# QEDProtocol/plonky2.5

Measured on AMD Instinct MI355X. Metric: recursive proofs/sec (fib-64 p3-in-p2 circuit), higher is better.
Workload: dtype u64 (Goldilocks, p = 2^64 - 2^32 + 1); 1 GPU; batch of 256 independent fib-64 plonky3-verifier proofs per GPU (n = 2^16 rows x 135 wires, LDE 2^19), 1 GPU(s), replicas + RCCL gather; all_statuses_ok=True, gathered_complete_and_ok=True, head=

## Files before the change

plonky2.5_amd/csrc/kernels.h:

```cpp
#pragma once
#include <hip/hip_runtime.h>
#include <stddef.h>
#include <stdint.h>
#include <stdexcept>
#include <string>
#include <vector>
#include <map>
#include <tuple>
#include "dev_res.h"
#include "gl.h"

#if defined(__HIP_DEVICE_COMPILE__)
#define P25_WAVE_PRIO(n) __builtin_amdgcn_s_setprio(n)
#else
#define P25_WAVE_PRIO(n) ((void)0)
#endif
#define P25_PRIO_BULK 2
#define P25_PRIO_CHAIN 3
namespace p25 {

void launch_poseidon_permute(u64* d_states, size_t n, hipStream_t st);
void launch_poseidon2_permute(u64* d_states, size_t n, hipStream_t st);
size_t merkle_tree_words(size_t n_leaves, unsigned cap_height);
size_t merkle_level_offset(size_t n_leaves, unsigned level);
u64* launch_merkle_tree(const u64* d_cols, size_t col_stride, int width, size_t n_leaves,
                        unsigned cap_height, u64* d_tree, hipStream_t st, hipEvent_t ev_begin = nullptr,
                        hipEvent_t ev_end = nullptr, bool single_proof = false);

struct NttPass {
  const u64* in;
  u64* out;
  size_t in_poly_stride, out_poly_stride;
  size_t coset_out_off[8];
  int log_r, log_nt, log_t;
  int in_kind, in_br_t, in_br_i;
  int out_kind, out_br_t, out_br_i;
  const u64* pow_table;
  int log_n_table;
  int use_twiddle;
  const u64* pre;
  const u64* pre_t;
  const u64* pre_i;
  const u64* post_t;
  const u64* post_i;
  int inverse;
  int lazy_out;
  uint32_t n_tiles, n_cosets, log_g, full_table;
};
void launch_ntt_pass(const NttPass& p, int n_polys, int n_cosets, hipStream_t st);
double measure_shader_clock_hz(hipStream_t st);

class NttTables {
 public:
  const u64* pow_table(int log_n, bool inverse);
  const u64* geom_table(u64 first, u64 ratio, size_t len);
  const u64* upload(const std::vector<u64>& host);
  typedef std::map<std::tuple<int, int, u64>, const u64*> CosetCache;
  CosetCache& coset_cache() { return coset_; }

 private:
  CosetCache coset_;
  std::map<std::pair<int, bool>, u64*> pow_;
  std::map<std::tuple<u64, u64, size_t>, u64*> geom_;
  std::vector<DevMem> owned_;
};

void ntt_inverse(NttTables& tb, const u64* d_in, size_t in_stride, bool in_bitrev, u64* d_tmp,
                 size_t tmp_stride, u64* d_out, size_t out_stride, int log_n, int n_polys,
                 u64 coset_shift, hipStream_t st);
void ntt_lde_bitrev(NttTables& tb, const u64* d_coeffs, size_t coeff_stride, u64* d_lde,
                    size_t lde_stride, int log_n, int rate_bits, int n_polys, u64 shift,
                    hipStream_t st);

void ntt_inverse_then_lde(NttTables& tb, const u64* d_vals, size_t val_stride, u64* d_tmp, size_t tmp_stride, u64* d_coeffs,
                          size_t coeff_stride, u64* d_lde, size_t lde_stride, int log_n, int rate_bits, int n_polys, u64 shift,
                          hipStream_t st);

}
```

plonky2.5_amd/csrc/kernels_fri.hip:

```cpp
#include "kernels.h"
#include "gl_lazy.h"
#include "coop.h"
#include "coop_lat.h"
#include "poseidon.h"
#include "prover_kernels.h"

namespace p25 {

constexpr uint32_t EXT_POW_MAX_JOBS = 5;
struct ExtPowJob {
  const u64* point;
  u64 scale;
  u64* out;
  uint32_t count, invert;
};
struct ExtPowJobs {
  ExtPowJob job[EXT_POW_MAX_JOBS];
};
__global__ void k_ext_pows(ExtPowJobs a) {
  P25_WAVE_PRIO(P25_PRIO_CHAIN);
  const ExtPowJob jb = a.job[blockIdx.y];
  uint32_t t = blockIdx.x * blockDim.x + threadIdx.x;
  if (t > jb.count) return;
  gl::E2 z = gl::mul(gl::E2{jb.point[0], jb.point[1]}, jb.scale);
// ... 138 lines not shown
  gl::E2 s0 = gl::e2(0);
  uint32_t j = 0;
  for (int o = 0; o < 4; o++)
    for (uint32_t p = 0; p < a.n_polys[o]; p++, j++) {
      u64 c = a.coeffs[o][(size_t)p * n + k];
      s0.a = gl::mad_nc(ap[2 * j], c, s0.a);
      s0.b = gl::mad_nc(ap[2 * j + 1], c, s0.b);
    }
  gl::E2 s1 = gl::e2(0);
  for (uint32_t c = 0; c < a.num_challenges; c++) {
    u64 v = a.coeffs[2][(size_t)c * n + k];
    s1.a = gl::mad_nc(ap[2 * c], v, s1.a);
    s1.b = gl::mad_nc(ap[2 * c + 1], v, s1.b);
  }
  gl::E2 d0 = gl::e2_canon(gl::e2_mul_nc(s0, gl::E2{a.zpow[0][2 * k], a.zpow[0][2 * k + 1]}));
  gl::E2 d1 = gl::e2_canon(gl::e2_mul_nc(s1, gl::E2{a.zpow[1][2 * k], a.zpow[1][2 * k + 1]}));
  a.comp[0 * (size_t)n + k] = d0.a;
  a.comp[1 * (size_t)n + k] = d0.b;
  a.comp[2 * (size_t)n + k] = d1.a;
  a.comp[3 * (size_t)n + k] = d1.b;
}

__global__ __launch_bounds__(256) void k_sfx_block(u64* data, uint32_t n, u64* block_tot) {
  P25_WAVE_PRIO(P25_PRIO_CHAIN);
  __shared__ u64 sh[256];
  u64* d = data + (size_t)blockIdx.y * n;
  uint32_t i = blockIdx.x * 256 + threadIdx.x;
  u64 v = i < n ? d[n - 1 - i] : 0;
  sh[threadIdx.x] = v;
  __syncthreads();
  for (int off = 1; off < 256; off <<= 1) {
    u64 t = threadIdx.x >= (unsigned)off ? sh[threadIdx.x - off] : 0;
    __syncthreads();
    v = gl::add(v, t);
    sh[threadIdx.x] = v;
    __syncthreads();
  }
  u64 ex = threadIdx.x == 0 ? 0 : sh[threadIdx.x - 1];
  if (i < n) d[n - 1 - i] = ex;
  if (threadIdx.x == 255) block_tot[(size_t)blockIdx.y * gridDim.x + blockIdx.x] = v;
}
__global__ __launch_bounds__(256) void k_sfx_totals(u64* block_tot, uint32_t n_blocks) {
  P25_WAVE_PRIO(P25_PRIO_CHAIN);
  __shared__ u64 sh[256];
  __shared__ u64 carry_s;
  u64* bt = block_tot + (size_t)blockIdx.x * n_blocks;
  if (threadIdx.x == 0) carry_s = 0;
  __syncthreads();
  for (uint32_t base = 0; base < n_blocks; base += 256) {
    uint32_t i = base + threadIdx.x;
    u64 v = i < n_blocks ? bt[i] : 0;
    sh[threadIdx.x] = v;
    __syncthreads();
    for (int off = 1; off < 256; off <<= 1) {
      u64 t = threadIdx.x >= (unsigned)off ? sh[threadIdx.x - off] : 0;
      __syncthreads();
      v = gl::add(v, t);
      sh[threadIdx.x] = v;
      __syncthreads();
    }
    u64 carry = carry_s;
    u64 excl = threadIdx.x == 0 ? carry : gl::add(carry, sh[threadIdx.x - 1]);
    __syncthreads();
    if (i < n_blocks) bt[i] = excl;
    if (threadIdx.x == 255) carry_s = gl::add(carry, v);
    __syncthreads();
  }
}
__global__ __launch_bounds__(256) void k_sfx_apply(u64* data, uint32_t n, const u64* block_tot) {
  P25_WAVE_PRIO(P25_PRIO_CHAIN);
  u64* d = data + (size_t)blockIdx.y * n;
  uint32_t i = blockIdx.x * 256 + threadIdx.x;
  if (i >= n) return;
  d[n - 1 - i] = gl::add(d[n - 1 - i], block_tot[(size_t)blockIdx.y * gridDim.x + blockIdx.x]);
}

__global__ __launch_bounds__(256) void k_fri_final(const u64* __restrict__ S, uint32_t n,
                                                   const u64* __restrict__ zinv0, const u64* __restrict__ zinv1,
                                                   const u64* __restrict__ alpha_pows, uint32_t nc,
                                                   u64* __restrict__ fa, u64* __restrict__ fb) {
  P25_WAVE_PRIO(P25_PRIO_CHAIN);
  uint32_t k = blockIdx.x * blockDim.x + threadIdx.x;
  if (k >= n) return;
  if (k == n - 1) {
    fa[0] = 0;
    fb[0] = 0;
    return;
  }
  gl::E2 q0 = gl::mul(gl::E2{S[k], S[(size_t)n + k]}, gl::E2{zinv0[2 * (k + 1)], zinv0[2 * (k + 1) + 1]});
  gl::E2 q1 = gl::mul(gl::E2{S[2 * (size_t)n + k], S[3 * (size_t)n + k]}, gl::E2{zinv1[2 * (k + 1)], zinv1[2 * (k + 1) + 1]});
  gl::E2 f = gl::add(gl::mul(q0, gl::E2{alpha_pows[2 * nc], alpha_pows[2 * nc + 1]}), q1);
  fa[k + 1] = f.a;
  fb[k + 1] = f.b;
}

void launch_fri_combine(const FriCombineArgs& a, hipStream_t st) {
  const uint32_t n = 1u << a.log_n;
  uint32_t total = a.n_polys[0] + a.n_polys[1] + a.n_polys[2] + a.n_polys[3];
  u64* alpha_pows = a.scan_tmp;
  u64* zpow0 = alpha_pows + 2 * (size_t)(total + 1);
  u64* zpow1 = zpow0 + 2 * (size_t)(n + 1);
  u64* zinv0 = zpow1 + 2 * (size_t)(n + 1);
  u64* zinv1 = zinv0 + 2 * (size_t)(n + 1);
  u64* block_tot = zinv1 + 2 * (size_t)(n + 1);
  const unsigned nb = (n + 255) / 256;
  ExtPowJobs pj{};
  pj.job[0] = ExtPowJob{a.chal + CH_FRI_ALPHA, (u64)1, alpha_pows, total, 0};
  pj.job[1] = ExtPowJob{a.chal + CH_ZETA, (u64)1, zpow0, n, 0};
  pj.job[2] = ExtPowJob{a.chal + CH_ZETA, a.g, zpow1, n, 0};
  pj.job[3] = ExtPowJob{a.chal + CH_ZETA, (u64)1, zinv0, n, 1};
  pj.job[4] = ExtPowJob{a.chal + CH_ZETA, a.g, zinv1, n, 1};
  launch_ext_pows(pj, 5, st);
  CombineK ck;
  for (int o = 0; o < 4; o++) {
    ck.coeffs[o] = a.coeffs[o];
    ck.n_polys[o] = a.n_polys[o];
  }
  ck.log_n = a.log_n;
  ck.num_challenges = a.num_challenges;
  ck.alpha_pows = alpha_pows;
  ck.zpow[0] = zpow0;
  ck.zpow[1] = zpow1;
  ck.comp = a.comp;
  hipLaunchKernelGGL(k_fri_comp, dim3(nb), dim3(256), 2 * total * sizeof(u64), st, ck);
  hipLaunchKernelGGL(k_sfx_block, dim3(nb, 4), dim3(256), 0, st, a.comp, n, block_tot);
  hipLaunchKernelGGL(k_sfx_totals, dim3(4), dim3(256), 0, st, block_tot, nb);
  hipLaunchKernelGGL(k_sfx_apply, dim3(nb, 4), dim3(256), 0, st, a.comp, n, block_tot);
  hipLaunchKernelGGL(k_fri_final, dim3(nb), dim3(256), 0, st, a.comp, n, zinv0, zinv1, alpha_pows, a.num_challenges, a.final_a, a.final_b);
}

__global__ __launch_bounds__(256) void k_fri_fold(const u64* __restrict__ ca, const u64* __restrict__ cb,
                                                  uint32_t len_out, uint32_t arity_bits,
                                                  const u64* __restrict__ beta, u64* __restrict__ oa,
                                                  u64* __restrict__ ob) {
  P25_WAVE_PRIO(P25_PRIO_BULK);
  uint32_t i = blockIdx.x * blockDim.x + threadIdx.x;
  if (i >= len_out) return;
  const uint32_t arity = 1u << arity_bits;
  gl::E2 b{beta[0], beta[1]};
  gl::E2 s = gl::e2(0);
  for (int k = (int)arity - 1; k >= 0; k--) {
    s = gl::mul(s, b);
    s = gl::add(s, gl::E2{ca[(size_t)i * arity + k], cb[(size_t)i * arity + k]});
  }
  oa[i] = s.a;
  ob[i] = s.b;
}
void launch_fri_fold(const u64* ca, const u64* cb, uint32_t len_out, uint32_t arity_bits, const u64* d_beta,
                     u64* oa, u64* ob, hipStream_t st) {
  hipLaunchKernelGGL(k_fri_fold, dim3((len_out + 255) / 256), dim3(256), 0, st, ca, cb, len_out, arity_bits, d_beta, oa, ob);
}

template <int PRIO>
__global__ __launch_bounds__(256) void k_fri_leaf_hash(const u64* __restrict__ va, const u64* __restrict__ vb,
                                                       uint32_t n_leaves, uint32_t arity_bits,
                                                       u64* __restrict__ digests) {
  if constexpr (PRIO != 0) P25_WAVE_PRIO(PRIO);
  uint32_t l = blockIdx.x * blockDim.x + threadIdx.x;
  if (l >= n_leaves) return;
  const uint32_t arity = 1u << arity_bits, words = 2 * arity;
  u64 s[12];
#pragma unroll
  for (int i = 0; i < 12; i++) s[i] = 0;
  u64 out[4];
  if (words <= 4) {
    for (uint32_t i = 0; i < 4; i++) out[i] = i < words ? ((i & 1) ? vb : va)[(size_t)l * arity + (i >> 1)] : 0;
  } else {
    for (uint32_t off = 0; off < words; off += 8) {
      uint32_t m = words - off < 8 ? words - off : 8;
      for (uint32_t i = 0; i < m; i++) {
        uint32_t wd = off + i;
        s[i] = ((wd & 1) ? vb : va)[(size_t)l * arity + (wd >> 1)];
      }
      poseidon::permute(s);
    }
    for (int i = 0; i < 4; i++) out[i] = s[i];
  }
  for (int i = 0; i < 4; i++) digests[4 * (size_t)l + i] = out[i];
}
__global__ __launch_bounds__(256) void k_fri_leaf_hash_coop(const u64* __restrict__ va, const u64* __restrict__ vb,
                                                            uint32_t n_leaves, uint32_t arity_bits,
                                                            u64* __restrict__ digests) {
  P25_WAVE_PRIO(P25_PRIO_CHAIN);
  __shared__ u64 rc_lds[360];
  coop::stage_poseidon_rc(rc_lds);
  size_t g = ((size_t)blockIdx.x * blockDim.x + threadIdx.x) / coop::GROUP;
  const int rr = threadIdx.x & (coop::GROUP - 1);
  const bool valid = g < n_leaves;
  if (!valid) g = n_leaves - 1;
  const uint32_t arity = 1u << arity_bits, words = 2 * arity;
  u64 s = 0;
  for (uint32_t off = 0; off < words; off += 8) {
    const uint32_t m = words - off < 8 ? words - off : 8;
    const uint32_t wd = off + (uint32_t)rr;
    if ((uint32_t)rr < m) s = ((wd & 1) ? vb : va)[g * arity + (wd >> 1)];
    s = coop::poseidon_permute_lat(s, threadIdx.x & 63, rc_lds);
  }
  if (valid && rr < 4) digests[4 * g + rr] = s;
}
constexpr uint32_t COOP_FRI_LEAVES_BATCH = 2048;
constexpr int FRI_LEAF_PRIO_BATCH = 1;
void launch_fri_leaf_hash(const u64* va, const u64* vb, uint32_t n_leaves, uint32_t arity_bits, u64* d_digests,
                          hipStream_t st, bool single_proof) {
  const bool noop = (2u << arity_bits) <= 4;
  if (single_proof ? noop : (noop || n_leaves > COOP_FRI_LEAVES_BATCH)) {
    if (single_proof)
      hipLaunchKernelGGL(k_fri_leaf_hash<0>, dim3((n_leaves + 255) / 256), dim3(256), 0, st, va, vb, n_leaves, arity_bits,
                         d_digests);
    else
      hipLaunchKernelGGL(k_fri_leaf_hash<FRI_LEAF_PRIO_BATCH>, dim3((n_leaves + 63) / 64), dim3(64), 0, st, va, vb, n_leaves,
                         arity_bits, d_digests);
    return;
  }
  const size_t th = (size_t)n_leaves * coop::GROUP;
  hipLaunchKernelGGL(k_fri_leaf_hash_coop, dim3((unsigned)((th + 255) / 256)), dim3(256), 0, st, va, vb, n_leaves,
                     arity_bits, d_digests);
}

__device__ __forceinline__ size_t level_off(size_t n_leaves, uint32_t k) { return 8 * n_leaves - ((8 * n_leaves) >> k); }

__global__ __launch_bounds__(256) void k_queries(QueryArgs a) {
  P25_WAVE_PRIO(P25_PRIO_CHAIN);
  const uint32_t q = blockIdx.x, t = threadIdx.x, nt = blockDim.x;
  const size_t big = (size_t)1 << a.lde_bits;
  size_t x = (size_t)(a.chal[CH_QUERIES + q] & (big - 1));
  u64* out = a.proof + a.query_offset + (size_t)q * a.query_stride;
  const uint32_t path_len = a.lde_bits - a.cap_height;
  for (uint32_t o = 0; o < a.n_oracles; o++) {
    for (uint32_t c = t; c < a.oracle_width[o]; c += nt) out[c] = a.oracle_lde[o][(size_t)c * big + x];
    out += a.oracle_width[o];
    for (uint32_t e = t; e < 4 * path_len; e += nt) {
      uint32_t k = e >> 2;
      out[e] = a.oracle_tree[o][level_off(big, k) + 4 * ((x >> k) ^ 1) + (e & 3)];
    }
    out += 4 * path_len;
  }
  uint32_t bits = a.lde_bits;
  for (uint32_t l = 0; l < a.n_layers; l++) {
    const uint32_t ab = a.arity_bits[l], arity = 1u << ab;
    bits -= ab;
    const size_t n_leaves = (size_t)1 << bits;
    const size_t ci = x >> ab;
    for (uint32_t e = t; e < 2 * arity; e += nt) out[e] = ((e & 1) ? a.layer_vb[l] : a.layer_va[l])[ci * arity + (e >> 1)];
    out += 2 * arity;
    const uint32_t pl = bits - a.cap_height;
    for (uint32_t e = t; e < 4 * pl; e += nt) {
      uint32_t k = e >> 2;
      out[e] = a.layer_tree[l][level_off(n_leaves, k) + 4 * ((ci >> k) ^ 1) + (e & 3)];
    }
    out += 4 * pl;
    x = ci;
  }
}
void launch_queries(const QueryArgs& a, hipStream_t st) {
  hipLaunchKernelGGL(k_queries, dim3(a.num_queries), dim3(256), 0, st, a);
}

}
```

plonky2.5_amd/csrc/kernels_quotient.hip:

```cpp
#include <stdexcept>
#include <stdlib.h>
#include "builder.h"
#include "kernels.h"
#include "gl_lazy.h"
#include "poseidon.h"
#include "poseidon2.h"
#include "coop.h"
#include "prover_kernels.h"

namespace p25 {

namespace {

struct AlphaLimbs {
  u32 l[8];
};
constexpr int MAX_TERMS_PER_FOLD = 512;

struct LaneCols {
  const u64* base;
  u32 boff;
  size_t big;
  typedef unsigned int u32x2 __attribute__((ext_vector_type(2)));
  __device__ __forceinline__ u64 col(size_t c) const {
// ... 371 lines not shown
  for (int copy = 0; copy < RA_COPIES; copy++) {
    const int base = (2 + RA_VEC) * copy;
    u64 bits[RA_BITS];
    for (int i = 0; i < RA_BITS; i++) {
      bits[i] = cx.w(RA_ROUTED + RA_BITS * copy + i);
      cx.at(nc++, gl::mul_nc(bits[i], gl::sub(bits[i], 1)));
    }
    u64 idx = 0;
    for (int i = RA_BITS - 1; i >= 0; i--) idx = gl::add(gl::add(idx, idx), bits[i]);
    cx.at(nc++, gl::sub(idx, cx.w(base)));
    u64 items[RA_VEC];
    for (int i = 0; i < RA_VEC; i++) items[i] = cx.w(base + 2 + i);
    int len = RA_VEC;
    for (int bi = 0; bi < RA_BITS; bi++) {
      len >>= 1;
      for (int i = 0; i < len; i++)
        items[i] = gl::add(items[2 * i], gl::mul(bits[bi], gl::sub(items[2 * i + 1], items[2 * i])));
    }
    cx.at(nc++, gl::sub(items[0], cx.w(base + 1)));
  }
  cx.at(nc++, gl::sub(k0, cx.w((2 + RA_VEC) * RA_COPIES)));
  cx.at(nc++, gl::sub(k1, cx.w((2 + RA_VEC) * RA_COPIES + 1)));
}
template <bool EXT>
__device__ void gate_reducing(Ctx& cx) {
  constexpr int NCO = EXT ? REDX_COEFFS : RED_COEFFS, CW = EXT ? 2 : 1, START_ACCS = 6 + NCO * CW;
  const gl::E2 alpha{cx.w(2), cx.w(3)};
  gl::E2 acc{cx.w(4), cx.w(5)};
  auto acc_wire = [](int i) { return i == NCO - 1 ? 0 : START_ACCS + 2 * i; };
  u64 na = cx.w(acc_wire(0)), nb = cx.w(acc_wire(0) + 1), nc0 = cx.w(6), nc1 = EXT ? cx.w(7) : 0;
  for (int i = 0; i < NCO; i++) {
    const gl::E2 nxt{na, nb};
    const u64 c0 = nc0, c1 = nc1;
    if (i + 1 < NCO) {
      na = cx.w(acc_wire(i + 1));
      nb = cx.w(acc_wire(i + 1) + 1);
      nc0 = cx.w(6 + CW * (i + 1));
      if (EXT) nc1 = cx.w(6 + CW * (i + 1) + 1);
    }
    gl::E2 t = gl::mul(acc, alpha);
    t.a = gl::add(t.a, c0);
    if (EXT) t.b = gl::add(t.b, c1);
    cx.at(2 * i, gl::sub(t.a, nxt.a));
    cx.at(2 * i + 1, gl::sub(t.b, nxt.b));
    acc = nxt;
  }
}
__device__ void gate_poseidon_mds(Ctx& cx) {
  for (int d = 0; d < 2; d++) {
    u64 in[12];
#pragma unroll
    for (int i = 0; i < 12; i++) in[i] = cx.w(2 * i + d);
    u64 nxt = cx.w(24 + d);
#pragma unroll
    for (int r = 0; r < 12; r++) {
      const u64 o = nxt;
      if (r + 1 < 12) nxt = cx.w(24 + 2 * (r + 1) + d);
      SmallLin acc;
#pragma unroll
      for (int i = 0; i < 12; i++) acc.add(in[(i + r) % 12], (u32)poseidon::MDS_CIRC[i] + (i == 0 && r == 0 ? (u32)poseidon::MDS_DIAG0 : 0u));
      cx.at(2 * r + d, gl::sub(o, gl::canon(acc.value())));
    }
  }
}
__device__ void gate_coset_interp(Ctx& cx) {
  const u64 shift = cx.w(0);
  const gl::E2 point{cx.w(CI_W_POINT), cx.w(CI_W_POINT + 1)}, x{cx.w(CI_W_SHIFTED), cx.w(CI_W_SHIFTED + 1)};
  int nc = 0;
  cx.at(nc++, gl::sub(point.a, gl::mul(x.a, shift)));
  cx.at(nc++, gl::sub(point.b, gl::mul(x.b, shift)));
  const u64 g = gl::root_of_unity(4), inv16 = gl::inv(16);
  gl::E2 eval{0, 0}, prod{1, 0};
  u64 xi = 1;
  for (int c = 0; c <= CI_INTER; c++) {
    if (c > 0) {
      const gl::E2 ie{cx.w(CI_W_INTER + 2 * (c - 1)), cx.w(CI_W_INTER + 2 * (c - 1) + 1)};
      const gl::E2 ip{cx.w(CI_W_INTER + 2 * (CI_INTER + c - 1)), cx.w(CI_W_INTER + 2 * (CI_INTER + c - 1) + 1)};
      cx.at(nc++, gl::sub(ie.a, eval.a));
      cx.at(nc++, gl::sub(ie.b, eval.b));
      cx.at(nc++, gl::sub(ip.a, prod.a));
      cx.at(nc++, gl::sub(ip.b, prod.b));
      eval = ie;
      prod = ip;
    }
    const int end = c == 0 ? CI_DEGREE : (1 + (CI_DEGREE - 1) * (c + 1) < CI_POINTS ? 1 + (CI_DEGREE - 1) * (c + 1) : CI_POINTS);
    for (int i = c == 0 ? 0 : 1 + (CI_DEGREE - 1) * c; i < end; i++) {
      const gl::E2 v = gl::mul(gl::E2{cx.w(1 + 2 * i), cx.w(2 + 2 * i)}, gl::mul(xi, inv16));
      const gl::E2 term{gl::sub(x.a, xi), x.b};
      eval = gl::add(gl::mul(eval, term), gl::mul(v, prod));
      prod = gl::mul(prod, term);
      xi = gl::mul(xi, g);
    }
  }
  cx.at(nc++, gl::sub(cx.w(CI_W_VALUE), eval.a));
  cx.at(nc++, gl::sub(cx.w(CI_W_VALUE + 1), eval.b));
}
__device__ void gate_poseidon(Ctx& cx) {
  int nc = 0;
  u64 swap = cx.w(24);
  cx.at(nc++, gl::mul_nc(swap, gl::sub(swap, 1)));
  u64 st[12];
#pragma unroll
  for (int i = 0; i < 4; i++) {
    u64 lhs = cx.w(i), rhs = cx.w(i + 4), delta = cx.w(25 + i);
    cx.at(nc++, gl::sub(gl::mul(swap, gl::sub(rhs, lhs)), delta));
    st[i] = gl::add(lhs, delta);
    st[i + 4] = gl::sub(rhs, delta);
  }
#pragma unroll
  for (int i = 8; i < 12; i++) st[i] = cx.w(i);
  int tr = 29;
  u64 nsb = cx.w(tr);
  constexpr int TR_END = 29 + 12 * (2 * poseidon::HALF_FULL - 1) + poseidon::N_PARTIAL;
  for (int r = 0; r < poseidon::N_ROUNDS; r++) {
#pragma unroll
    for (int i = 0; i < 12; i++) st[i] = poseidon::add_rc(st[i], poseidon::RC[12 * r + i]);
    if (r < poseidon::HALF_FULL || r >= poseidon::HALF_FULL + poseidon::N_PARTIAL) {
      if (r != 0) {
#pragma unroll
        for (int i = 0; i < 12; i++) {
          const u64 sb = nsb;
          tr++;
          if (tr < TR_END) nsb = cx.w(tr);
          cx.at(nc++, gl::sub(gl::canon(st[i]), sb));
          st[i] = sb;
        }
      }
#pragma unroll
      for (int i = 0; i < 12; i++) st[i] = poseidon::sbox(st[i]);
    } else {
      const u64 sb = nsb;
      tr++;
      if (tr < TR_END) nsb = cx.w(tr);
      cx.at(nc++, gl::sub(gl::canon(st[0]), sb));
      st[0] = poseidon::sbox(sb);
    }
    poseidon::mds(st);
  }
#pragma unroll
  for (int i = 0; i < 12; i++) cx.at(nc++, gl::sub(gl::canon(st[i]), cx.w(12 + i)));
}

}

__global__ void k_alpha_pows(const u64* __restrict__ chal, u64* __restrict__ out) {
  P25_WAVE_PRIO(P25_PRIO_CHAIN);
  int c = blockIdx.x, j = threadIdx.x;
  if (j < ALPHA_POWS) out[c * ALPHA_POWS + j] = gl::pow(chal[CH_ALPHAS + c], (u64)j);
}
void launch_alpha_pows(const u64* d_chal, u64* d_alpha_pows, hipStream_t st) {
  hipLaunchKernelGGL(k_alpha_pows, dim3(2), dim3(ALPHA_POWS), 0, st, d_chal, d_alpha_pows);
}

constexpr int Q_WAVES = 4;
constexpr int QREC_WAVES = 3;
constexpr int Q_PF = 1;
template <bool REC>
__device__ __forceinline__ void quotient_body(const QuotientArgs& a) {
  __shared__ u64 ap[2 * ALPHA_POWS];
  __shared__ AlphaLimbs apl[ALPHA_POWS];
  for (int i = threadIdx.x; i < 2 * ALPHA_POWS; i += blockDim.x) {
    const u64 v = a.alpha_pows[i];
    ap[i] = v;
    const int ch = i / ALPHA_POWS, j = i - ch * ALPHA_POWS;
    apl[j].l[4 * ch] = (u32)v & 0x3FFFFFu;
    apl[j].l[4 * ch + 1] = (u32)(v >> 22) & 0x3FFFFFu;
    apl[j].l[4 * ch + 2] = (u32)(v >> 44);
    apl[j].l[4 * ch + 3] = 0;
  }
  __shared__ u64 kb[2 * MAX_ROUTED];
  for (int i = threadIdx.x; i < 2 * (int)a.num_routed; i += blockDim.x) {
    const int c = i / (int)a.num_routed, j = i - c * (int)a.num_routed;
    kb[i] = gl::mul(a.k_is[j], a.chal[CH_BETAS + c]);
  }
  __syncthreads();
  const uint32_t lde_bits = a.degree_bits + a.rate_bits;
  const size_t big = (size_t)1 << lde_bits;
  const size_t p = (size_t)blockIdx.x * blockDim.x + threadIdx.x;
  if (p >= big) return;
  const uint32_t i_nat = gl::bitrev((u32)p, lde_bits);
  const u64 x = gl::mul(gl::GENERATOR, a.pow_big[i_nat]);
  const uint32_t rate_mask = (1u << a.rate_bits) - 1;
  const u64 zhx = a.zh[i_nat & rate_mask], zhi = a.zh_inv[i_nat & rate_mask];
  const uint32_t i_next = (i_nat + (1u << a.rate_bits)) & (uint32_t)(big - 1);
  const size_t p_next = gl::bitrev(i_next, lde_bits);

  const int NC = 2, NP = (int)a.num_partial_products, RW = (int)a.num_routed;
  const int nch = NP + 1, per = (int)a.quotient_degree_factor;
  const u32 boff = (u32)p * 8u;
  const LaneCols csc{a.cs_lde, boff, big}, wrc{a.wires_lde, boff, big}, zsc{a.zs_lde, boff, big};
  const int n_consts = (int)a.num_selectors;

  u64 res[2] = {0, 0};
  {
    u64 l0 = gl::mul_nc(zhx, a.l0_inv[p]);
    for (int c = 0; c < NC; c++) {
      u64 t = gl::mul_nc(l0, gl::sub_c(zsc.col(c), 1));
      res[0] = gl::mad_nc(t, ap[c], res[0]);
      res[1] = gl::mad_nc(t, ap[ALPHA_POWS + c], res[1]);
    }
  }
  auto gate_filter = [&](uint32_t gi) {
    const GateEntry ge = a.gates[gi];
    const u64 s = csc.col(ge.selector_index);
    u64 filter = 1;
    for (uint32_t k = ge.group_start; k < ge.group_end; k++)
      if (k != gi) filter = gl::mul_nc(filter, gl::sub_c((u64)k, s));
    if (a.num_selectors > 1) filter = gl::mul_nc(filter, gl::sub_c(0xFFFFFFFFull, s));
    return filter;
  };
  const bool fast = per == 8 && RW == 80 && NP == 9 && a.num_wires >= 80;
  uint32_t merged_mask = 0;
  u64 mg0 = 0, mg1 = 0;
  const u64 beta0 = a.chal[CH_BETAS], beta1 = a.chal[CH_BETAS + 1];
  const u64 gamma0 = a.chal[CH_GAMMAS], gamma1 = a.chal[CH_GAMMAS + 1];
  if (fast) {
    for (uint32_t gi = 0; gi < a.n_gates; gi++) {
      const uint32_t kind = a.gates[gi].kind;
      if (kind == G_CONSTANT || kind == G_PUBLIC_INPUT || kind == G_BASE_SUM || kind == G_ARITHMETIC || kind == G_MUL_EXT) {
        if ((merged_mask >> kind) & 1u) { merged_mask = 0xFFFFFFFFu; break; }
        merged_mask |= 1u << kind;
      }
    }
  }
  if (fast && merged_mask != 0xFFFFFFFFu) {
    const bool h_const = (merged_mask >> G_CONSTANT) & 1u, h_pi = (merged_mask >> G_PUBLIC_INPUT) & 1u,
               h_bsum = (merged_mask >> G_BASE_SUM) & 1u, h_arith = (merged_mask >> G_ARITHMETIC) & 1u,
               h_mext = (merged_mask >> G_MUL_EXT) & 1u;
    u64 f_const = 0, f_pi = 0, f_bsum = 0, f_arith = 0, f_mext = 0;
    for (uint32_t gi = 0; gi < a.n_gates; gi++) {
      const uint32_t kind = a.gates[gi].kind;
      if (kind == G_CONSTANT) f_const = gate_filter(gi);
      else if (kind == G_PUBLIC_INPUT) f_pi = gate_filter(gi);
      else if (kind == G_BASE_SUM) f_bsum = gate_filter(gi);
      else if (kind == G_ARITHMETIC) f_arith = gate_filter(gi);
      else if (kind == G_MUL_EXT) f_mext = gate_filter(gi);
    }
    const u64 k0 = csc.col(n_consts), k1 = csc.col(n_consts + 1);
    Ctx mc;
    mc.wires = wrc;
    mc.big = big;
    mc.apl = apl;
    mc.reset();
    u64 bs_sum = 0, bs_w0 = 0;
    u64 wnext = wrc.col(0);
    SmallLin bs_acc;
    u64 ar0 = 0, ar1 = 0, ar2 = 0;
    u64 mx0 = 0, mx1 = 0, mx2 = 0, mx3 = 0, mx4 = 0;
#define P25_Q_WIRE(JJ)                                                                                          \
  {                                                                                                             \
    const int j = base + (JJ);                                                                                  \
    const u64 w = wnext;                                                                                        \
    if (j + 1 < 80) wnext = wrc.col(j + 1);                                                                      \
    if ((JJ) < 4 && base == 0) {                                                                                \
      if (h_const && (JJ) < 2) mc.at((JJ), gl::mul_nc(gl::sub_c((JJ) == 0 ? k0 : k1, w), f_const));            \
      if (h_pi) mc.at((JJ), gl::mul_nc(gl::sub_c(w, a.pi_hash[(JJ)]), f_pi));                                   \
    }                                                                                                           \
    if (h_bsum) {                                                                                               \
      if (j == 0) bs_w0 = w;                                                                                    \
      if (j >= 1 && j <= BASE_SUM_LIMBS) {                                                                      \
        constexpr int t = ((JJ) + 7) % 8;             \
        bs_acc.add(w, 1u << t);                                                                                 \
        mc.at(j, gl::mul_nc(bool01(w), f_bsum));                                                                \
        if (t == 7 || j == BASE_SUM_LIMBS) {                                                                    \
          bs_sum = gl::mad_nc(bs_acc.value(), (u64)1 << (8 * (((j - 1) >> 3) & 7)), bs_sum);                          \
          bs_acc = SmallLin();                                                                                  \
        }                                                                                                       \
      }                                                                                                         \
    }                                                                                                           \
    if (h_arith) {                                                                                              \
      if ((JJ) % 4 == 0) ar0 = w;                                                                               \
      else if ((JJ) % 4 == 1) ar1 = w;                                                                          \
      else if ((JJ) % 4 == 2) ar2 = w;                                                                          \
      else {                                                                                                    \
        const u64 comp = gl::mad_nc(gl::mul_nc(ar0, ar1), k0, gl::mul_nc(ar2, k1));                             \
        mc.at(j >> 2, gl::mul_nc(gl::sub_nc(w, comp), f_arith));                                                \
      }                                                                                                         \
    }                                                                                                           \
    if (h_mext && j < 78) {                                                                                     \
      if ((JJ) % 6 == 0) mx0 = w;                                                                               \
      else if ((JJ) % 6 == 1) mx1 = w;                                                                          \
      else if ((JJ) % 6 == 2) mx2 = w;                                                                          \
      else if ((JJ) % 6 == 3) mx3 = w;                                                                          \
      else if ((JJ) % 6 == 4) mx4 = w;                                                                          \
      else {                                                                                                    \
        const gl::E2 pr = e2_mul_scaled(gl::E2{mx0, mx1}, gl::E2{mx2, mx3}, k0);                                \
        const int op = j / 6;                                                                                   \
        mc.at(2 * op, gl::mul_nc(gl::sub_nc(mx4, pr.a), f_mext));                                               \
        mc.at(2 * op + 1, gl::mul_nc(gl::sub_nc(w, pr.b), f_mext));                                             \
      }                                                                                                         \
    }                                                                                                           \
  }
#define P25_Q_WIRES8(J0) P25_Q_WIRE(J0) P25_Q_WIRE(J0 + 1) P25_Q_WIRE(J0 + 2) P25_Q_WIRE(J0 + 3) \
                         P25_Q_WIRE(J0 + 4) P25_Q_WIRE(J0 + 5) P25_Q_WIRE(J0 + 6) P25_Q_WIRE(J0 + 7)
    for (int base = 0; base < 72; base += 24) {
      P25_Q_WIRES8(0) P25_Q_WIRES8(8) P25_Q_WIRES8(16)
    }
    {
      const int base = 72;
      P25_Q_WIRES8(0)
    }
#undef P25_Q_WIRES8
#undef P25_Q_WIRE
    if (h_bsum) mc.at(0, gl::mul_nc(gl::sub_c(bs_sum, bs_w0), f_bsum));
    mg0 = mc.acc0();
    mg1 = mc.acc1();
  } else {
// ... 140 lines not shown
```

plonky2.5_amd/csrc/kernels_transcript.hip:

```cpp
#include "kernels.h"
#include "coop.h"
#include "prover_kernels.h"

namespace p25 {

using coop::shfl64;

struct Sponge {
  u64 state, inb, outb;
  uint32_t n_in, n_out;
  int lane;
  const u64* rc;
  __device__ void duplex() {
    if (lane < (int)n_in) state = inb;
    n_in = 0;
    state = coop::poseidon_permute_single(state, lane, rc);
    outb = state;
    n_out = 8;
  }
  __device__ void observe(u64 x) {
    n_out = 0;
    if (lane == (int)n_in) inb = x;
    n_in++;
    if (n_in == 8) duplex();
  }
  __device__ u64 challenge() {
    if (n_in > 0 || n_out == 0) duplex();
    u64 v = shfl64(outb, (int)n_out - 1);
    n_out--;
    return v;
  }
};

__global__ __launch_bounds__(64) void k_transcript(Transcript* tr, TranscriptArgs a) {
  P25_WAVE_PRIO(P25_PRIO_CHAIN);
  __shared__ u64 rc_lds[360];
  coop::stage_poseidon_rc(rc_lds);
  const int lane = threadIdx.x;
  Sponge sp;
  sp.lane = lane;
  sp.rc = rc_lds;
  if (a.init) {
    sp.state = 0;
    sp.inb = 0;
    sp.outb = 0;
    sp.n_in = 0;
    sp.n_out = 0;
  } else {
    sp.state = lane < 12 ? tr->state[lane] : 0;
    sp.inb = lane < 8 ? tr->in[lane] : 0;
    sp.outb = lane < 8 ? tr->out[lane] : 0;
    sp.n_in = tr->n_in;
    sp.n_out = tr->n_out;
  }
  u64 w0 = 0;
  for (uint32_t s = 0; s < a.n_seg; s++) {
    const TrSegment sg = a.seg[s];
    for (uint32_t base = 0; base < sg.n_words; base += 64) {
      const uint32_t cnt = sg.n_words - base < 64 ? sg.n_words - base : 64;
      u64 v = 0;
      if ((uint32_t)lane < cnt) {
        const uint32_t i = base + (uint32_t)lane;
        v = sg.src_b ? ((i & 1) ? sg.src_b : sg.src)[i >> 1] : sg.src[i];
        if (sg.copy_dst) sg.copy_dst[i] = v;
      }
      if (s == 0 && base == 0) w0 = shfl64(v, 0);
      for (uint32_t j = 0; j < cnt; j++) sp.observe(shfl64(v, (int)j));
    }
  }
  u64 c0 = 0, c1 = 0;
  for (uint32_t i = 0; i < a.n_chal; i++) {
    u64 c = sp.challenge();
    if (i == 0) c0 = c;
    if (i == 1) c1 = c;
    if (lane == 0) a.chal_out[i] = c;
  }
  if (lane < 12) tr->state[lane] = sp.state;
  if (lane < 8) {
    tr->in[lane] = sp.inb;
    tr->out[lane] = sp.outb;
  }
  if (lane == 0) {
    tr->n_in = sp.n_in;
    tr->n_out = sp.n_out;
  }
  switch (a.close) {
    case TR_CLOSE_ALPHA_POWS: {
      for (int c = 0; c < 2; c++) {
        const u64 al = c ? c1 : c0, al64 = gl::pow(al, 64);
        u64 p = gl::pow(al, (u64)lane);
        for (int j = lane; j < ALPHA_POWS; j += 64) {
          a.close_out[c * ALPHA_POWS + j] = p;
          p = gl::mul(p, al64);
        }
      }
      break;
    }
    case TR_CLOSE_CHECK_ZETA: {
      gl::E2 zn = gl::exp_pow2(gl::E2{c0, c1}, a.close_arg);
      if (lane == 0 && zn.a == 1 && zn.b == 0) set_status(a.status, 6);
      break;
    }
    case TR_CLOSE_POW_INIT:
      if (lane == 0) *a.close_out = ~0ull;
      break;
    case TR_CLOSE_FINISH:
      if (lane == 0 && (w0 == ~0ull || (uint32_t)__clzll((long long)c0) < a.close_arg)) set_status(a.status, 7);
      break;
    default:
      break;
  }
}

void launch_transcript(Transcript* d_tr, const TranscriptArgs& a, hipStream_t st) {
  if (a.n_seg > TR_MAX_SEGMENTS) throw std::invalid_argument("too many transcript segments in one launch");
  hipLaunchKernelGGL(k_transcript, dim3(1), dim3(64), 0, st, d_tr, a);
}
void launch_transcript(Transcript* d_tr, int init, const u64* d_obs, uint32_t n_obs, u64* d_chal_out,
                       uint32_t n_chal, hipStream_t st) {
  TranscriptArgs a{};
  a.seg[0] = TrSegment{d_obs, nullptr, nullptr, n_obs};
  a.n_seg = 1;
  a.init = (uint32_t)init;
  a.chal_out = d_chal_out;
  a.n_chal = n_chal;
  launch_transcript(d_tr, a, st);
}

template <int PRIO>
__global__ __launch_bounds__(256) void k_pow_search(const Transcript* __restrict__ tr, uint32_t pow_bits, u64 total,
                                                    u64* result) {
  if constexpr (PRIO != 0) P25_WAVE_PRIO(PRIO);
  const u64 G = (u64)gridDim.x * blockDim.x;
  for (u64 cand = (u64)blockIdx.x * blockDim.x + threadIdx.x; cand < total; cand += G) {
    if (__hip_atomic_load(result, __ATOMIC_RELAXED, __HIP_MEMORY_SCOPE_AGENT) < cand) return;
    u64 s[12];
#pragma unroll
    for (int i = 0; i < 12; i++) s[i] = tr->state[i];
    const uint32_t pos = tr->n_in;
    for (uint32_t i = 0; i < pos; i++) s[i] = tr->in[i];
#pragma unroll
    for (int i = 0; i < 8; i++)
      if ((uint32_t)i == pos) s[i] = cand;
    poseidon::permute(s);
    if ((uint32_t)__clzll((long long)s[7]) >= pow_bits) atomicMin((unsigned long long*)result, (unsigned long long)cand);
  }
}

__global__ __launch_bounds__(64) void k_public_inputs(const u64* __restrict__ vals, size_t B, uint32_t p,
                                                      const uint32_t* __restrict__ pi_slots, uint32_t n,
                                                      u64* __restrict__ values_out, u64* __restrict__ hash_out) {
  P25_WAVE_PRIO(P25_PRIO_CHAIN);
  __shared__ u64 rc_lds[360];
  coop::stage_poseidon_rc(rc_lds);
  const int lane = threadIdx.x;
  u64 s = 0;
  for (uint32_t off = 0; off < n; off += 8) {
    if (lane < 8 && off + lane < n) {
      s = vals[(size_t)pi_slots[off + lane] * B + p];
      values_out[off + lane] = s;
    }
    s = coop::poseidon_permute_single(s, lane, rc_lds);
  }
  if (lane < 4) hash_out[lane] = s;
}
void launch_public_inputs(const u64* d_vals, size_t B, uint32_t p, const uint32_t* d_pi_slots, uint32_t n, u64* d_values_out,
                          u64* d_hash_out, hipStream_t st) {
  hipLaunchKernelGGL(k_public_inputs, dim3(1), dim3(64), 0, st, d_vals, B, p, d_pi_slots, n, d_values_out, d_hash_out);
}

constexpr int POW_PRIO_BATCH = 1;
void launch_pow_search(const Transcript* d_tr, int pow_bits, u64* d_result, hipStream_t st, bool single_proof) {
  const int wb = pow_bits < 12 ? 12 : pow_bits;
  const int gb = wb < 16 ? wb : 16;
  const dim3 grid(1u << (gb - 8));
  const u64 total = (u64)1 << (wb + 6);
  if (single_proof)
    hipLaunchKernelGGL(k_pow_search<0>, grid, dim3(256), 0, st, d_tr, (uint32_t)pow_bits, total, d_result);
  else
    hipLaunchKernelGGL(k_pow_search<POW_PRIO_BATCH>, grid, dim3(256), 0, st, d_tr, (uint32_t)pow_bits, total, d_result);
}

}
```

plonky2.5_amd/csrc/kernels_zpp.hip:

```cpp
#include "kernels.h"
#include "gl_lazy.h"
#include "prover_kernels.h"

namespace p25 {


__global__ __launch_bounds__(256) void k_zpp_chunks(ZppArgs a) {
  P25_WAVE_PRIO(P25_PRIO_BULK);
  uint32_t r = blockIdx.x * blockDim.x + threadIdx.x;
  uint32_t c = blockIdx.y;
  if (r >= a.n) return;
  const u64 beta = a.chal[CH_BETAS + c], gamma = a.chal[CH_GAMMAS + c];
  const u64 x = a.pow_n[r];
  const int nch = (int)a.num_partial_products + 1;
  const int per = (int)a.quotient_degree_factor;
  u64 num[MAX_CHUNKS], den[MAX_CHUNKS];
  for (int k = 0; k < nch; k++) {
    u64 np = 1, dp = 1;
    for (int j = k * per; j < (k + 1) * per && j < (int)a.num_routed; j++) {
      const u64 wg = gl::add_c(a.wires[(size_t)j * a.n + r], gamma);
      const u64 nu = gl::mad_nc(beta, gl::mul_nc(a.k_is[j], x), wg);
      const u64 de = gl::mad_nc(beta, a.sigmas[(size_t)j * a.n + r], wg);
      np = gl::mul_nc(np, nu);
      dp = gl::mul_nc(dp, de);
    }
    num[k] = gl::canon(np);
    den[k] = gl::canon(dp);
  }
  u64 pre[MAX_CHUNKS];
  u64 acc = 1;
  for (int k = 0; k < nch; k++) {
    pre[k] = acc;
    acc = gl::mul(acc, den[k]);
  }
  u64 inv = gl::inv(acc);
  u64 tot = 1;
  u64 q[MAX_CHUNKS];
  for (int k = nch - 1; k >= 0; k--) {
    u64 di = gl::mul(inv, pre[k]);
    inv = gl::mul(inv, den[k]);
    q[k] = gl::mul(num[k], di);
  }
  for (int k = 0; k < nch; k++) {
    a.chunk[((size_t)c * nch + k) * a.n + r] = q[k];
    tot = gl::mul(tot, q[k]);
  }
  a.tot[(size_t)c * a.n + r] = tot;
}

__global__ __launch_bounds__(256) void k_zpp_scan_block(ZppArgs a) {
  P25_WAVE_PRIO(P25_PRIO_CHAIN);
  __shared__ u64 sh[256];
  uint32_t c = blockIdx.y, r = blockIdx.x * 256 + threadIdx.x;
  u64 v = r < a.n ? a.tot[(size_t)c * a.n + r] : 1;
  sh[threadIdx.x] = v;
  __syncthreads();
  for (int off = 1; off < 256; off <<= 1) {
    u64 t = threadIdx.x >= (unsigned)off ? sh[threadIdx.x - off] : 1;
    __syncthreads();
    v = gl::mul(v, t);
    sh[threadIdx.x] = v;
    __syncthreads();
  }
  if (r < a.n) a.tot[(size_t)c * a.n + r] = v;
  if (threadIdx.x == 255) a.block_tot[(size_t)c * gridDim.x + blockIdx.x] = v;
}
__global__ __launch_bounds__(256) void k_zpp_scan_totals(u64* block_tot, uint32_t n_blocks) {
  P25_WAVE_PRIO(P25_PRIO_CHAIN);
  __shared__ u64 sh[256];
  __shared__ u64 carry_s;
  u64* bt = block_tot + (size_t)blockIdx.x * n_blocks;
  if (threadIdx.x == 0) carry_s = 1;
  __syncthreads();
  for (uint32_t base = 0; base < n_blocks; base += 256) {
    uint32_t i = base + threadIdx.x;
    u64 orig = i < n_blocks ? bt[i] : 1;
    u64 v = orig;
    sh[threadIdx.x] = v;
    __syncthreads();
    for (int off = 1; off < 256; off <<= 1) {
      u64 t = threadIdx.x >= (unsigned)off ? sh[threadIdx.x - off] : 1;
      __syncthreads();
      v = gl::mul(v, t);
      sh[threadIdx.x] = v;
      __syncthreads();
    }
    u64 carry = carry_s;
    u64 excl = threadIdx.x == 0 ? carry : gl::mul(carry, sh[threadIdx.x - 1]);
    __syncthreads();
    if (i < n_blocks) bt[i] = excl;
    if (threadIdx.x == 255) carry_s = gl::mul(carry, v);
    __syncthreads();
  }
}
__global__ __launch_bounds__(256) void k_zpp_finish(ZppArgs a) {
  P25_WAVE_PRIO(P25_PRIO_CHAIN);
  uint32_t c = blockIdx.y, r = blockIdx.x * 256 + threadIdx.x;
  if (r >= a.n) return;
  const int NP = (int)a.num_partial_products, nch = NP + 1;
  u64 z = a.block_tot[(size_t)c * gridDim.x + blockIdx.x];
  if (threadIdx.x > 0) z = gl::mul(z, a.tot[(size_t)c * a.n + r - 1]);
  a.out[(size_t)c * a.n + r] = z;
  u64 acc = z;
  for (int k = 0; k < NP; k++) {
    acc = gl::mul(acc, a.chunk[((size_t)c * nch + k) * a.n + r]);
    a.out[((size_t)a.num_challenges + (size_t)c * NP + k) * a.n + r] = acc;
  }
}

void launch_zpp(const ZppArgs& a, hipStream_t st) {
  dim3 grid((a.n + 255) / 256, a.num_challenges);
  hipLaunchKernelGGL(k_zpp_chunks, grid, dim3(256), 0, st, a);
  hipLaunchKernelGGL(k_zpp_scan_block, grid, dim3(256), 0, st, a);
  hipLaunchKernelGGL(k_zpp_scan_totals, dim3(a.num_challenges), dim3(256), 0, st, a.block_tot, grid.x);
  hipLaunchKernelGGL(k_zpp_finish, grid, dim3(256), 0, st, a);
}

}
```

Before: 140.2 proofs/s.

## Split zpp chunk products across grid, cap waves for sponge kernels, retune pow search

Splits the permutation partial-product chunk computation so each thread handles one chunk, with chunk index on the grid. Numerators and denominators are stored separately, and the batch inversion and per-row product move into the block-scan kernel, which now walks 256 rows in 64-lane segments carrying a running product. Separately, it adds an amdgpu_waves_per_eu hint to the prioritised FRI leaf-hash and PoW kernels, raises Q_WAVES from 4 to 5, and launches batch PoW search as 64-thread blocks. These target occupancy and register pressure, trading extra global traffic (the denominators round-trip through the out buffer) and more scan-side serial work.

```diff
diff --git a/plonky2.5_amd/csrc/kernels.h b/plonky2.5_amd/csrc/kernels.h
--- a/plonky2.5_amd/csrc/kernels.h
+++ b/plonky2.5_amd/csrc/kernels.h
@@ -9,6 +9,8 @@
 #include <tuple>
 #include "dev_res.h"
 #include "gl.h"
+
+#define P25_WAVES_BESIDE_SPONGES(PRIO) __attribute__((amdgpu_waves_per_eu((PRIO) != 0 ? 5 : 1, (PRIO) != 0 ? 5 : 8)))
 
 #if defined(__HIP_DEVICE_COMPILE__)
 #define P25_WAVE_PRIO(n) __builtin_amdgcn_s_setprio(n)
diff --git a/plonky2.5_amd/csrc/kernels_fri.hip b/plonky2.5_amd/csrc/kernels_fri.hip
--- a/plonky2.5_amd/csrc/kernels_fri.hip
+++ b/plonky2.5_amd/csrc/kernels_fri.hip
@@ -314,7 +314,7 @@
 }
 
 template <int PRIO>
-__global__ __launch_bounds__(256) void k_fri_leaf_hash(const u64* __restrict__ va, const u64* __restrict__ vb,
+__global__ __launch_bounds__(256) P25_WAVES_BESIDE_SPONGES(PRIO) void k_fri_leaf_hash(const u64* __restrict__ va, const u64* __restrict__ vb,
                                                        uint32_t n_leaves, uint32_t arity_bits,
                                                        u64* __restrict__ digests) {
   if constexpr (PRIO != 0) P25_WAVE_PRIO(PRIO);
diff --git a/plonky2.5_amd/csrc/kernels_quotient.hip b/plonky2.5_amd/csrc/kernels_quotient.hip
--- a/plonky2.5_amd/csrc/kernels_quotient.hip
+++ b/plonky2.5_amd/csrc/kernels_quotient.hip
@@ -547,7 +547,7 @@
   hipLaunchKernelGGL(k_alpha_pows, dim3(2), dim3(ALPHA_POWS), 0, st, d_chal, d_alpha_pows);
 }
 
-constexpr int Q_WAVES = 4;
+constexpr int Q_WAVES = 5;
 constexpr int QREC_WAVES = 3;
 constexpr int Q_PF = 1;
 template <bool REC>
diff --git a/plonky2.5_amd/csrc/kernels_transcript.hip b/plonky2.5_amd/csrc/kernels_transcript.hip
--- a/plonky2.5_amd/csrc/kernels_transcript.hip
+++ b/plonky2.5_amd/csrc/kernels_transcript.hip
@@ -128,7 +128,7 @@
 }
 
 template <int PRIO>
-__global__ __launch_bounds__(256) void k_pow_search(const Transcript* __restrict__ tr, uint32_t pow_bits, u64 total,
+__global__ __launch_bounds__(256) P25_WAVES_BESIDE_SPONGES(PRIO) void k_pow_search(const Transcript* __restrict__ tr, uint32_t pow_bits, u64 total,
                                                     u64* result) {
   if constexpr (PRIO != 0) P25_WAVE_PRIO(PRIO);
   const u64 G = (u64)gridDim.x * blockDim.x;
@@ -173,12 +173,12 @@
 void launch_pow_search(const Transcript* d_tr, int pow_bits, u64* d_result, hipStream_t st, bool single_proof) {
   const int wb = pow_bits < 12 ? 12 : pow_bits;
   const int gb = wb < 16 ? wb : 16;
-  const dim3 grid(1u << (gb - 8));
   const u64 total = (u64)1 << (wb + 6);
   if (single_proof)
-    hipLaunchKernelGGL(k_pow_search<0>, grid, dim3(256), 0, st, d_tr, (uint32_t)pow_bits, total, d_result);
+    hipLaunchKernelGGL(k_pow_search<0>, dim3(1u << (gb - 8)), dim3(256), 0, st, d_tr, (uint32_t)pow_bits, total, d_result);
   else
-    hipLaunchKernelGGL(k_pow_search<POW_PRIO_BATCH>, grid, dim3(256), 0, st, d_tr, (uint32_t)pow_bits, total, d_result);
+    hipLaunchKernelGGL(k_pow_search<POW_PRIO_BATCH>, dim3(1u << (gb - 6)), dim3(64), 0, st, d_tr, (uint32_t)pow_bits, total,
+                       d_result);
 }
 
 }
diff --git a/plonky2.5_amd/csrc/kernels_zpp.hip b/plonky2.5_amd/csrc/kernels_zpp.hip
--- a/plonky2.5_amd/csrc/kernels_zpp.hip
+++ b/plonky2.5_amd/csrc/kernels_zpp.hip
@@ -4,66 +4,80 @@
 
 namespace p25 {
 
+constexpr uint32_t ZPP_LANES = 64;
+constexpr uint32_t ZPP_SCAN_ROWS = 256;
 
-__global__ __launch_bounds__(256) void k_zpp_chunks(ZppArgs a) {
+__global__ __launch_bounds__(ZPP_LANES) void k_zpp_chunks(ZppArgs a) {
   P25_WAVE_PRIO(P25_PRIO_BULK);
-  uint32_t r = blockIdx.x * blockDim.x + threadIdx.x;
-  uint32_t c = blockIdx.y;
+  const uint32_t r = blockIdx.x * ZPP_LANES + threadIdx.x;
+  const uint32_t k = blockIdx.y, c = blockIdx.z;
   if (r >= a.n) return;
   const u64 beta = a.chal[CH_BETAS + c], gamma = a.chal[CH_GAMMAS + c];
   const u64 x = a.pow_n[r];
-  const int nch = (int)a.num_partial_products + 1;
-  const int per = (int)a.quotient_degree_factor;
-  u64 num[MAX_CHUNKS], den[MAX_CHUNKS];
-  for (int k = 0; k < nch; k++) {
-    u64 np = 1, dp = 1;
-    for (int j = k * per; j < (k + 1) * per && j < (int)a.num_routed; j++) {
-      const u64 wg = gl::add_c(a.wires[(size_t)j * a.n + r], gamma);
-      const u64 nu = gl::mad_nc(beta, gl::mul_nc(a.k_is[j], x), wg);
-      const u64 de = gl::mad_nc(beta, a.sigmas[(size_t)j * a.n + r], wg);
-      np = gl::mul_nc(np, nu);
-      dp = gl::mul_nc(dp, de);
-    }
-    num[k] = gl::canon(np);
-    den[k] = gl::canon(dp);
+  const uint32_t per = a.quotient_degree_factor;
+  const uint32_t j0 = k * per, j1 = (k + 1) * per < a.num_routed ? (k + 1) * per : a.num_routed;
+  u64 np = 1, dp = 1;
+#pragma unroll 1
+  for (uint32_t j = j0; j < j1; j++) {
+    const u64 wg = gl::add_c(a.wires[(size_t)j * a.n + r], gamma);
+    const u64 nu = gl::mad_nc(beta, gl::mul_nc(a.k_is[j], x), wg);
+    const u64 de = gl::mad_nc(beta, a.sigmas[(size_t)j * a.n + r], wg);
+    np = gl::mul_nc(np, nu);
+    dp = gl::mul_nc(dp, de);
   }
-  u64 pre[MAX_CHUNKS];
-  u64 acc = 1;
-  for (int k = 0; k < nch; k++) {
-    pre[k] = acc;
-    acc = gl::mul(acc, den[k]);
-  }
-  u64 inv = gl::inv(acc);
-  u64 tot = 1;
-  u64 q[MAX_CHUNKS];
-  for (int k = nch - 1; k >= 0; k--) {
-    u64 di = gl::mul(inv, pre[k]);
-    inv = gl::mul(inv, den[k]);
-    q[k] = gl::mul(num[k], di);
-  }
-  for (int k = 0; k < nch; k++) {
-    a.chunk[((size_t)c * nch + k) * a.n + r] = q[k];
-    tot = gl::mul(tot, q[k]);
-  }
-  a.tot[(size_t)c * a.n + r] = tot;
+  const size_t col = ((size_t)c * (a.num_partial_products + 1) + k) * a.n + r;
+  a.chunk[col] = gl::canon(np);
+  a.out[col] = gl::canon(dp);
 }
 
-__global__ __launch_bounds__(256) void k_zpp_scan_block(ZppArgs a) {
+__global__ __launch_bounds__(ZPP_LANES) void k_zpp_scan_block(ZppArgs a) {
   P25_WAVE_PRIO(P25_PRIO_CHAIN);
-  __shared__ u64 sh[256];
-  uint32_t c = blockIdx.y, r = blockIdx.x * 256 + threadIdx.x;
-  u64 v = r < a.n ? a.tot[(size_t)c * a.n + r] : 1;
-  sh[threadIdx.x] = v;
+  __shared__ u64 pre[MAX_CHUNKS][ZPP_LANES];
+  __shared__ u64 sh[ZPP_LANES];
+  __shared__ u64 carry_s;
+  const uint32_t c = blockIdx.y, t = threadIdx.x;
+  const int nch = (int)a.num_partial_products + 1;
+  u64* nq = a.chunk + (size_t)c * nch * a.n;
+  const u64* den = a.out + (size_t)c * nch * a.n;
+  if (t == 0) carry_s = 1;
+#pragma unroll 1
+  for (uint32_t seg = 0; seg < ZPP_SCAN_ROWS; seg += ZPP_LANES) {
+    const uint32_t r = blockIdx.x * ZPP_SCAN_ROWS + seg + t;
+    u64 v = 1;
+    if (r < a.n) {
+      u64 acc = 1;
+#pragma unroll 1
+      for (int k = 0; k < nch; k++) {
+        pre[k][t] = acc;
+        acc = gl::mul(acc, den[(size_t)k * a.n + r]);
+      }
+      u64 inv = gl::inv(acc);
+#pragma unroll 1
+      for (int k = nch - 1; k >= 0; k--) {
+        const u64 q = gl::mul(nq[(size_t)k * a.n + r], gl::mul(inv, pre[k][t]));
+        nq[(size_t)k * a.n + r] = q;
+        __builtin_amdgcn_sched_barrier(0);
+        v = gl::mul(v, q);
+        __builtin_amdgcn_sched_barrier(0);
+        inv = gl::mul(inv, den[(size_t)k * a.n + r]);
+      }
+    }
+    sh[t] = v;
+    __syncthreads();
+    for (uint32_t off = 1; off < ZPP_LANES; off <<= 1) {
+      u64 u = t >= off ? sh[t - off] : 1;
+      __syncthreads();
+      v = gl::mul(v, u);
+      sh[t] = v;
+      __syncthreads();
+    }
+    const u64 carry = carry_s;
+    if (r < a.n) a.tot[(size_t)c * a.n + r] = gl::mul(v, carry);
+    __syncthreads();
+    if (t == ZPP_LANES - 1) carry_s = gl::mul(v, carry);
+  }
   __syncthreads();
-  for (int off = 1; off < 256; off <<= 1) {
-    u64 t = threadIdx.x >= (unsigned)off ? sh[threadIdx.x - off] : 1;
-    __syncthreads();
-    v = gl::mul(v, t);
-    sh[threadIdx.x] = v;
-    __syncthreads();
-  }
-  if (r < a.n) a.tot[(size_t)c * a.n + r] = v;
-  if (threadIdx.x == 255) a.block_tot[(size_t)c * gridDim.x + blockIdx.x] = v;
+  if (t == 0) a.block_tot[(size_t)c * gridDim.x + blockIdx.x] = carry_s;
 }
 __global__ __launch_bounds__(256) void k_zpp_scan_totals(u64* block_tot, uint32_t n_blocks) {
   P25_WAVE_PRIO(P25_PRIO_CHAIN);
@@ -109,9 +123,11 @@
 }
 
 void launch_zpp(const ZppArgs& a, hipStream_t st) {
-  dim3 grid((a.n + 255) / 256, a.num_challenges);
-  hipLaunchKernelGGL(k_zpp_chunks, grid, dim3(256), 0, st, a);
-  hipLaunchKernelGGL(k_zpp_scan_block, grid, dim3(256), 0, st, a);
+  static_assert(ZPP_SCAN_ROWS == 256, "k_zpp_scan_totals / k_zpp_finish index block_tot by 256-row blocks");
+  const uint32_t nch = a.num_partial_products + 1;
+  dim3 grid((a.n + ZPP_SCAN_ROWS - 1) / ZPP_SCAN_ROWS, a.num_challenges);
+  hipLaunchKernelGGL(k_zpp_chunks, dim3((a.n + ZPP_LANES - 1) / ZPP_LANES, nch, a.num_challenges), dim3(ZPP_LANES), 0, st, a);
+  hipLaunchKernelGGL(k_zpp_scan_block, grid, dim3(ZPP_LANES), 0, st, a);
   hipLaunchKernelGGL(k_zpp_scan_totals, dim3(a.num_challenges), dim3(256), 0, st, a.block_tot, grid.x);
   hipLaunchKernelGGL(k_zpp_finish, grid, dim3(256), 0, st, a);
 }
```

Measured after the change: 141.5 proofs/s (median of 6 runs). Within noise of the previous version (+0.9%).
